# THU-DA-6D-Pose-Group/GDR-Net

Hardware: AMD Instinct MI355X
Metric: RoI crops/sec (fwd+bwd) at 256×256 bs=64 (higher is better)
Workload: dtype bf16; 1 GPU; LM-13 a6_cPnP_lm13 graph: ResNet-34 + RotWithRegionHead + ConvPnPNet, 256x256 RoIs, bs=64/GPU, train step: fwd + 8 losses + bwd + fused Ranger optimizer step (all inside the timed region); global_batch=64, parallelism=dp1

## Files before the change

### gdr-net_amd/cabi.py

```python
import ctypes as C
import os

_HERE = os.path.dirname(os.path.abspath(__file__))
LIB_PATH = os.environ.get("GDRN_HIP_LIB") or os.path.join(_HERE, "lib", "libgdrn_hip.so")
LIB_PATH_F16 = os.environ.get("GDRN_HIP_LIB_F16") or os.path.join(_HERE, "lib", "libgdrn_hip_f16.so")

F32, BF16, F16 = 0, 1, 2
PREZEROED = 0x100
ACC_ROWS = 0x200
P = C.c_void_p
I = C.c_int
LL = C.c_longlong
F = C.c_float
D = C.c_double


class GdrnHipError(RuntimeError):
    pass


class ConvParams(C.Structure):
    _fields_ = [
        ("x", P), ("w", P), ("y", P), ("bias", P), ("addend", P), ("stats", P),
        ("bnb_x", P), ("bnb_mask", P), ("bnb_mean", P), ("bnb_invstd", P), ("bnb_scale", P), ("bnb_shift", P), ("bnb_rows", P),
# ... 128 lines not shown
    "gdrn_stem_conv_pool": [P, P, P, P, P, I, I, P],
    "gdrn_head_conv_tail_fwd": [P, I, P, I, P, P, P, P, I, P, I, I, I, I, I, P],
    "gdrn_head_conv_tail_loss_rows": [I, I],
    "gdrn_head_out_dgrad_rows": [I, I],
    "gdrn_head_out_dgrad": [P, I, P, I, P, I, P, P, P, P, P, I, P, I, I, I, P],
    "gdrn_head_conv_tail_loss_fwd": [P, I, P, I, P, P, P, P, I, P, I, P, P, P, P, P, I, I, I, I, P],
    "gdrn_stem_wgrad_parts": [I],
    "gdrn_stem_wgrad": [P, P, P, P, P, P, I, P, P, I, P],
    "gdrn_linear_splitk": [P, P, P, P, I, I, I, I, I, I, I, P, I, P],
    "gdrn_conv_tile": [C.POINTER(ConvParams), C.POINTER(I), C.POINTER(I)],
    "gdrn_conv_stats_rows": [C.POINTER(ConvParams)],
    "gdrn_pack_wfrag": [P, P, I, I, I, P],
    "gdrn_pack_wfrag32": [P, P, I, I, I, P],
    "gdrn_conv3x3_wfrag": [C.POINTER(ConvParams)],
    "gdrn_conv3x3_halo": [C.POINTER(ConvParams), P],
    "gdrn_conv3x3_tile": [C.POINTER(ConvParams), C.POINTER(I), C.POINTER(I), C.POINTER(I)],
    "gdrn_conv3x3_stats_rows": [C.POINTER(ConvParams)],
    "gdrn_conv3x3_halo_waves": [C.POINTER(ConvParams)],
    "gdrn_conv_wgrad": [C.POINTER(WgradParams), P],
    "gdrn_conv3x3_wgrad": [C.POINTER(WgradParams), P],
    "gdrn_conv3x3_wgrad_ok": [C.POINTER(WgradParams)],
    "gdrn_conv3x3_wgrad_splits": [C.POINTER(WgradParams)],
    "gdrn_conv3x3_wgrad_multi": [P, P, I, I, P],
    "gdrn_conv3x3_wgrad_multi_lds": [P, P, I, I, I, P],
    "gdrn_wgrad_reduce_multi": [P, P, I, I, P],
    "gdrn_pack4": [P, P, I, I, I, I, I, I, I, LL, LL, LL, LL, I, I, P],
    "gdrn_unpack4": [P, P, I, I, I, I, I, I, I, LL, LL, LL, LL, I, P],
    "gdrn_pack_stem_w": [P, P, I, P],
    "gdrn_unpack_stem_w": [P, P, P],
    "gdrn_pack_image": [P, P, I, I, I, I, I, I, P],
    "gdrn_cast_from_f32": [P, P, LL, I, P],
    "gdrn_cast_to_f32": [P, P, LL, I, P],
    "gdrn_nhwc_to_nchw_f32": [P, I, I, I, P, I, I, I, P],
    "gdrn_bn_finalize": [P, I, I, D, P, P, P, P, P, F, F, P, P, P, P, P, P],
    "gdrn_bn_eval_params": [P, P, P, P, F, I, P, P, P],
    "gdrn_bn_apply": [P, P, P, P, P, LL, I, I, I, P],
    "gdrn_bn_bwd_reduce_rows": [LL, I, I],
    "gdrn_bn_bwd_reduce": [P, P, P, P, P, P, P, LL, I, P, I, P],
    "gdrn_bn_bwd_coef": [P, I, I, LL, P, P, P, P, P, P, P, P, P],
    "gdrn_bn_bwd_apply": [P, P, P, P, P, P, P, P, LL, I, P, P, I, P],
    "gdrn_bn_relu_maxpool_fwd": [P, P, P, P, P, I, I, I, I, I, P],
    "gdrn_maxpool_bwd_rows": [I, I, I, I, I],
    "gdrn_maxpool_bwd": [P, P, P, P, P, P, I, I, I, I, P, P, P, I, P],
    "gdrn_upsample2x_fwd": [P, P, I, I, I, I, I, P],
    "gdrn_upsample2x_bwd": [P, P, I, I, I, I, I, P],
    "gdrn_conv3x3s2_ok": [C.POINTER(S2Params)],
    "gdrn_conv3x3s2_stats_rows": [C.POINTER(S2Params)],
    "gdrn_conv3x3s2": [C.POINTER(S2Params), P],
    "gdrn_conv3x3s2_dgrad_ok": [C.POINTER(S2dParams)],
    "gdrn_conv3x3s2_dgrad_rows": [C.POINTER(S2dParams)],
    "gdrn_conv3x3s2_dgrad": [C.POINTER(S2dParams), P],
    "gdrn_block64_eval_ok": [I, I, I, I],
    "gdrn_block64_eval": [P, P, P, P, P, P, I, I, I, I, P],
    "gdrn_bn_relu_upsample2x_fwd": [P, P, P, P, I, I, I, I, I, P],
    "gdrn_upsample2x_bwd_bnsums": [P, P, P, P, P, P, P, I, I, I, I, P, I, P],
    "gdrn_gn_relu_fwd": [P, P, P, P, P, I, I, I, I, F, I, P],
    "gdrn_gn_relu_bwd": [P, P, P, P, P, P, P, P, I, I, I, I, I, P],
    "gdrn_leaky_bwd": [P, P, P, LL, I, P],
    "gdrn_bias_grad": [P, I, I, I, P, I, P],
    "gdrn_head_tail_fwd": [P, I, P, P, P, I, I, I, I, I, P],
    "gdrn_head_tail_loss_fwd": [P, I, P, P, P, I, P, P, P, P, P, I, I, I, I, P],
    "gdrn_map_loss_fwd": [P, I, P, P, P, P, I, I, I, P, P],
    "gdrn_map_loss_finalize": [P, I, I, P, P],
    "gdrn_head_tail_loss_rows": [I, I, I, I, I],
    "gdrn_map_loss_finalize_rows": [P, I, I, I, P, P],
    "gdrn_loss_finalize": [P, I, I, I, P, P, P, P, P],
    "gdrn_linear_splits": [I, I],
    "gdrn_head_tail_bwd": [P, I, P, P, I, P, P, P, P, P, P, P, P, I, I, I, I, I, P],
    "gdrn_pose_loss": [C.POINTER(PoseParams), P],
    "gdrn_combine3": [P, P, P, I, P],
    "gdrn_ranger_step": [P, P, P, P, P, I, I, I, F, F, F, F, F, F, I, I, F, P],
    "gdrn_pack_chunk": [],
    "gdrn_zero_chunk": [],
    "gdrn_zero_multi": [P, P, I, I, P],
    "gdrn_nonfinite_flag": [P, LL, P, P],
    "gdrn_pack_multi": [P, P, I, I, I, P],
    "gdrn_pack_transpose_blocks": [P],
    "gdrn_unpack_multi": [P, P, I, I, P],
    "gdrn_ranger_multi": [P, P, I, I, F, F, F, F, F, I, I, F, F, P],
    "gdrn_ranger_multi_dyn": [P, P, I, I, F, F, F, F, I, I, F, F, P, P],
    "gdrn_loss_scale_update": [P, I, P],
    "gdrn_unscale_or_zero": [P, LL, F, P, P],
    "gdrn_scaled_loss_weights": [P, P, I, P, P, P],
    "gdrn_roi_affine": [P, I, I, I, P, P, P, P, P],
    "gdrn_roi_crop_inputs": [P, P, I, I, I, C.POINTER(D), C.POINTER(D), P, P, P],
    "gdrn_roi_targets": [P, P, I, I, P, I, P, P, P, P, P, P, P],
    "gdrn_pose_metrics_workspace_bytes": [I, I],
    "gdrn_pose_errors": [P, P, P, P, P, P, P, I, P, P, I, P, P, P, I, I, P, P, P],
    "gdrn_pose_recall_accumulate": [P, P, P, I, P, I, P, P, P, P, P, P],
    "gdrn_pnp_workspace_bytes": [I, I, I],
    "gdrn_pnp_ransac": [P, P, P, P, P, I, I, D, I, C.c_ulonglong, I, P, P, P, P, P, P, P, P],
    "gdrn_pnp_refine": [P, P, P, P, P, I, I, I, P, P, P, P, P, P],
    "gdrn_pnp_ransac_f64": [P, P, P, P, P, I, I, D, I, C.c_ulonglong, I, P, P, P, P, P, P, P, P],
    "gdrn_pnp_refine_f64": [P, P, P, P, P, I, I, I, P, P, P, P, P, P],
    "gdrn_render_depth": [P, P, P, P, P, P, I, I, P, P, P, P, P, I, I, I, D, D, P, P],
    "gdrn_xyz_from_depth": [P, P, P, P, I, I, I, P, P, P, P, P],
    "gdrn_vsd_workspace_bytes": [I, I, I, I],
    "gdrn_vsd": [P, P, P, P, P, I, P, P, I, I, I, D, P, I, I, I, P, P, P, P],
    "gdrn_mssd_mspd_workspace_bytes": [I, I, I],
    "gdrn_mssd_mspd": [P, P, P, P, P, P, P, I, P, P, I, P, P, P, I, I, P, P, P],
    "gdrn_bop_recall_accumulate": [P, I, P, P, P, I, P, I, D, P, P, P, P, P, P, P, P],
    "gdrn_ad_errors_workspace_bytes": [I, I],
    "gdrn_ad_errors": [P, P, P, P, P, P, I, P, P, I, I, P, P, P],
    "gdrn_sym_errors_workspace_bytes": [I, I, I],
    "gdrn_sym_errors": [P, P, P, P, P, P, P, I, P, P, I, P, P, P, I, I, P, P, P],
    "gdrn_score_recall_accumulate": [P, P, P, P, I, P, P, I, P, P, P],
    "gdrn_aug_mask_cuts": [P, C.POINTER(AugTask), I, P, P],
    "gdrn_aug_frames": [P, C.POINTER(AugTask), I, P, LL, P, P],
    "gdrn_rle_decode": [P, C.POINTER(RleTask), I, P, LL, P, LL, P, P, P],
    "gdrn_rle_count": [P, C.POINTER(RleTask), I, P, LL, P, P, P],
    "gdrn_rle_positions": [P, C.POINTER(RleTask), I, P, LL, P, P, LL, P],
    "gdrn_rle_string": [P, C.POINTER(RleTask), I, P, P, LL, P, P, LL, P, P],
    "gdrn_model_prep_workspace_bytes": [I, I, I],
    "gdrn_model_bounds": [P, P, P, I, I, P, P],
    "gdrn_model_fps": [P, P, P, I, I, I, P, P, P, P],
    "gdrn_model_diameter": [P, P, P, I, I, P, P],
    "gdrn_scene_gt_canvas": [P, I, I, I, I, I, P, P, P, P],
    "gdrn_scene_gt_compose": [P, P, P, P, P, I, I, I, I, P, P],
    "gdrn_scene_gt_visibility": [P, P, P, P, I, P, I, I, I, D, I, P, P, P, P, P, P, P, P, P],
    "gdrn_render_visibility": [P, P, P, P, P, P, I, I, P, P, P, P, P, I, I, I, D, D, P, P],
    "gdrn_shade_frames": [P, P, P, P, P, P, P, P, P, I, P, P, P, P, P, P, P, P, P, I, I, I, I, P, P, P, P, P, P, P, P, P],
    "gdrn_shade_frames_tex": [P, P, P, P, P, P, P, P, P, P, P, P, P, I, I, P, P, P, P, P, P, P, P, P, I, I, I, I, P, P, I, I, P, P, P, P, P, P, P],
}

_SIGS["gdrn_half_format"] = []
_RET_LL = ("gdrn_workspace_bytes", "gdrn_pose_metrics_workspace_bytes", "gdrn_pnp_workspace_bytes", "gdrn_vsd_workspace_bytes",
           "gdrn_mssd_mspd_workspace_bytes", "gdrn_model_prep_workspace_bytes", "gdrn_ad_errors_workspace_bytes",
           "gdrn_sym_errors_workspace_bytes")
EXPORTS = tuple(_SIGS.keys())
_libs = {}


def lib_path(dtype=BF16):
    return LIB_PATH_F16 if dtype == F16 else LIB_PATH


def load(dtype=BF16):
    kind = F16 if dtype == F16 else BF16
    if kind in _libs:
        return _libs[kind]
    import torch

    path = lib_path(kind)
    if not os.path.exists(path):
        raise GdrnHipError(
            f"{path} not found: build it with `python -c 'import __graft_entry__ as g; g.build()'` "
            "(hipcc --offload-arch=gfx950).  There is no CPU fallback for the product path."
        )
    lib = C.CDLL(path)
    for name, args in _SIGS.items():
        fn = getattr(lib, name)
        fn.argtypes = args
        fn.restype = LL if name in _RET_LL else I
    if lib.gdrn_half_format() != kind:
        raise GdrnHipError(f"{path} computes 16-bit dtype code {lib.gdrn_half_format()}, expected {kind}")
    _libs[kind] = lib
    return lib


def check(status, what=""):
    if status != 0:
        names = {-1: "invalid argument", -2: "unsupported shape", -3: "launch failure"}
        detail = ""
        if status == -3:
            for lib in _libs.values():
                buf = C.create_string_buffer(64)
                code = lib.gdrn_last_hip_error(buf, 64)
                if code:
                    detail = f" (HIP error {code}: {buf.value.decode(errors='replace')})"
                    break
        raise GdrnHipError(f"libgdrn_hip: {what} failed: {names.get(status, status)}{detail}")


def ptr(t):
    return None if t is None else t.data_ptr()
```

### gdr-net_amd/csrc/conv3x3_halo.hip

```cpp
#include <hip/amd_detail/amd_hip_unsafe_atomics.h>

#include <algorithm>
#include <cstdlib>
#include <mutex>

#include "common.h"
#include "halo_xf.h"
#include "../../include/gdrn_hip.h"

namespace {

constexpr int ROWB = 128;

__device__ __forceinline__ f32x4_t mma_f32(uint4 a, uint4 b, f32x4_t c, int ks_) {
    const unsigned av = ks_ == 0 ? a.x : (ks_ == 1 ? a.y : (ks_ == 2 ? a.z : a.w));
    const unsigned bv = ks_ == 0 ? b.x : (ks_ == 1 ? b.y : (ks_ == 2 ? b.z : b.w));
    return __builtin_amdgcn_mfma_f32_16x16x4f32(__uint_as_float(av), __uint_as_float(bv), c, 0, 0, 0);
}

template <typename T>
__global__ __launch_bounds__(256) void pack_wfrag_kernel(const T* __restrict__ src, T* __restrict__ dst, int rows, int Cin) {
    constexpr int EPS = ROWB / (int)sizeof(T);
    constexpr int GE = 16 / (int)sizeof(T);
    const int kch = Cin / EPS;
    const long long total = (long long)rows * 9 * Cin / GE;
    for (long long i = (long long)blockIdx.x * blockDim.x + threadIdx.x; i < total; i += (long long)gridDim.x * blockDim.x) {
        const int lane = (int)(i & 63);
        long long r = i >> 6;
        const int ks = (int)(r & 1); r >>= 1;
        const int kc = (int)(r % kch); r /= kch;
        const int tap = (int)(r % 9);
        const int cb = (int)(r / 9);
        const int FNp = (rows <= 64 || sizeof(T) == 4) ? 1 : 2, rr = lane & 15;
        const int co = (cb / FNp) * 16 * FNp + (rr >> 2) * (4 * FNp) + (cb % FNp) * 4 + (rr & 3), g = lane >> 4;
        const size_t so = ((size_t)(co * 9 + tap) * Cin + (size_t)kc * EPS) + (size_t)(ks * 4 + g) * GE;
        *reinterpret_cast<uint4*>(dst + i * GE) = *reinterpret_cast<const uint4*>(src + so);
    }
}

#ifdef HALO_DBG
__device__ unsigned long long* g_halo_dbg;
__device__ __forceinline__ unsigned long long halo_clock() {
    unsigned long long t;
    asm volatile("s_memtime %0\n\ts_waitcnt lgkmcnt(0)" : "=s"(t)::"memory");
    return t;
}
struct HaloDbg {
    unsigned long long t[6] = {0, 0, 0, 0, 0, 0};
    int slot, lane;
    __device__ ~HaloDbg() {
        t[4] = halo_clock();
        asm volatile("s_waitcnt vmcnt(0)" ::: "memory");
        t[5] = halo_clock();
        if (lane == 0 && g_halo_dbg)
            for (int i = 0; i < 6; ++i) g_halo_dbg[(size_t)slot * 8 + i] = t[i];
    }
};
extern "C" int gdrn_halo_set_dbg(unsigned long long* buf) { return hipMemcpyToSymbol(HIP_SYMBOL(g_halo_dbg), &buf, sizeof(buf)) == hipSuccess ? 0 : -3; }
#define HALO_STAMP(i_) hdbg_.t[i_] = halo_clock();
#else
#define HALO_STAMP(i_)
#endif

template <typename T, int TH, int TW, int BN, int XF, int KS = 1>
__global__ __launch_bounds__(256 * KS, KS == 2 ? 1 : ((BN == 64 && TW == 16 && sizeof(T) == 2) ? 3 : 2)) void conv3x3_halo_kernel(const gdrn_conv_params p) {
    static_assert(KS == 1 || (KS == 2 && sizeof(T) == 2 && BN == 128), "the 8-wave form: 16-bit, 128-channel tile");
    constexpr int EPS = ROWB / (int)sizeof(T);
    constexpr int BM = TH * TW;
    constexpr int PW = TW + 2, PH = TH + 2, PPIX = PH * PW;
    constexpr int HB = half_bytes(PPIX);
    constexpr int PBYTES = 2 * HB;
    constexpr int PSEG = PPIX * 8;
    constexpr int PSLICE = XF ? ((PSEG + 8) / 9 + 7) / 8 * 8 : (PSEG + 8) / 9;
    static_assert(PSLICE <= 256, "one patch segment per thread per stage");
    static_assert(XF == 0 || sizeof(T) == 2, "operand transforms are bf16 only");
    constexpr int FM = BM / 16;
    constexpr int FN = BN / 64;
    constexpr int WQ = FN * 2 / KS;
    constexpr int NSL = KS == 2 ? 5 : 9;
    extern __shared__ __attribute__((aligned(16))) unsigned char smem[];

    const int lane = threadIdx.x & 63;
    const int grp = KS == 2 ? __builtin_amdgcn_readfirstlane((int)threadIdx.x >> 8) : 0;
    const int tid = threadIdx.x & 255, wave = tid >> 6;
    const int g = lane >> 4, r16 = lane & 15;
#ifdef HALO_DBG
    HaloDbg hdbg_;
    hdbg_.slot = (int)blockIdx.x * 4 + wave;
    hdbg_.lane = lane;
#endif
    HALO_STAMP(0)
    __builtin_amdgcn_s_setprio(2);

    const int NTn = (p.Cout + BN - 1) / BN;
    int bid = blockIdx.x;
    {
        const int nwg = gridDim.x, q = nwg >> 3, r = nwg & 7, xcd = bid & 7, j = bid >> 3;
        bid = (xcd < r ? xcd * (q + 1) : r * (q + 1) + (xcd - r) * q) + j;
    }
    const int nt = bid % NTn;
    const int mt = bid / NTn;
    int t = mt;
    const int tiles_x = p.Wo / TW, tiles_y = p.Ho / TH;
    const int tx = t % tiles_x; t /= tiles_x;
    const int ty = t % tiles_y;
    const int n = t / tiles_y;
    const int co0 = nt * BN;
    const int y0 = ty * TH, x0 = tx * TW;

    const int kch = p.Cin / EPS;
    const char* xg = reinterpret_cast<const char*>(p.x);
    const int cb0 = (co0 + wave * (BN / 4)) / 16;
    const char* wl = reinterpret_cast<const char*>(p.w) + (size_t)lane * 16 + (size_t)(grp << 10);

    auto wptr = [&](int kc, int tap, int a, int ks) -> const uint4* {
        return reinterpret_cast<const uint4*>(wl + ((size_t)((((cb0 + a) * 9 + tap) * kch + kc) * 2 + ks) << 10));
    };
    uint4 wq0[WQ], wq1[WQ], wq2[WQ];

#define LOADW(dst, kc_, tap_)                                                   \
    {                                                                           \
        _Pragma("unroll") for (int a_ = 0; a_ < FN; ++a_) {                     \
            if constexpr (KS == 1) {                                            \
                dst[a_ * 2 + 0] = *wptr(kc_, tap_, a_, 0);                      \
                dst[a_ * 2 + 1] = *wptr(kc_, tap_, a_, 1);                      \
            } else dst[a_] = *wptr(kc_, tap_, a_, 0);                           \
        }                                                                       \
    }
    LOADW(wq0, 0, 0) LOADW(wq1, 0, 1) LOADW(wq2, 0, 2)

    unsigned poff[NSL];
    int pdst[NSL];
    unsigned pokm = 0, pinm = 0, ppm = 0;
#pragma unroll
    for (int sj = 0; sj < NSL; ++sj) {
        const int st = KS == 2 ? 2 * sj + grp : sj;
        const int id = st * PSLICE + tid;
        const int pp = id >> 3, sg = id & 7;
        const int py = pp / PW, px = pp - py * PW;
        const int iy = y0 + py - 1, ix = x0 + px - 1;
        const bool inpatch = tid < PSLICE && id < PSEG && st < 9;
        const bool ok = inpatch && iy >= 0 && iy < p.Hi && ix >= 0 && ix < p.Wi;
        const int iyc = min(max(iy, 0), p.Hi - 1), ixc = min(max(ix, 0), p.Wi - 1);
        poff[sj] = (unsigned)((n * p.Hi + iyc) * p.Wi + ixc) * (unsigned)p.x_cs * (unsigned)sizeof(T) + sg * 16;
        pdst[sj] = inpatch ? (pp * HALF_PITCH + (sg & 1) * HB + (sg >> 1) * 16) : -1;
        pokm |= ok ? (1u << sj) : 0u;
        if constexpr (XF != 0) {
            pinm |= (inpatch && py >= 1 && py <= TH && px >= 1 && px <= TW) ? (1u << sj) : 0u;
            ppm |= inpatch ? (1u << sj) : 0u;
        }
    }
    constexpr int PDSTEP = (PSLICE / 8) * HALF_PITCH;
    const int pdst0 = (tid >> 3) * HALF_PITCH + (tid & 1) * HB + ((tid & 7) >> 1) * 16 + grp * PDSTEP;
#define OWN(st_) (KS == 1 || (((st_) & 1) == grp))
#define SJ(st_) (KS == 1 ? (st_) : ((st_) >> 1))
    const float* xtab = nullptr;
    const char* xg2 = nullptr;
    char* xo = nullptr;
    float xlo = 0.f;
    if constexpr (XF != 0) {
        float* tabw = reinterpret_cast<float*>(smem + (kch == 1 ? 1 : 2) * PBYTES);
        for (int c = (int)threadIdx.x; c < p.Cin; c += 256 * KS) {
            tabw[c] = p.xf_a ? p.xf_a[c] : 1.f;
            tabw[p.Cin + c] = p.xf_c[c];
            if constexpr (XF >= 2) tabw[2 * p.Cin + c] = p.xf_b ? p.xf_b[c] : 1.f;
            if constexpr (XF == 2) tabw[3 * p.Cin + c] = p.xf_c2 ? p.xf_c2[c] : 0.f;
            if constexpr (XF == 4) { tabw[3 * p.Cin + c] = p.xf_msc[c]; tabw[4 * p.Cin + c] = p.xf_msh[c]; }
        }
        xtab = tabw + (tid & 7) * 8;
        xg2 = reinterpret_cast<const char*>(p.xf_x2);
        xo = (nt == 0) ? reinterpret_cast<char*>(p.xf_out) : nullptr;
        xlo = p.xf_relu ? 0.f : -__builtin_inff();
    }

    int lbase;
    if constexpr (TW == 16) lbase = r16 * HALF_PITCH + (g & 1) * HB + (g >> 1) * 16;
    else lbase = ((r16 >> 3) * PW + (r16 & 7)) * HALF_PITCH + (g & 1) * HB + (g >> 1) * 16;
    lbase += grp * 32;
    constexpr int FROW = (TW == 16) ? PW * HALF_PITCH : 2 * PW * HALF_PITCH;

    f32x4_t acc[FN][FM];
#pragma unroll
    for (int a = 0; a < FN; ++a)
#pragma unroll
        for (int b = 0; b < FM; ++b) acc[a][b] = f32x4_t{0.f, 0.f, 0.f, 0.f};
    f32x4_t part[sizeof(T) == 4 ? FN : 1][sizeof(T) == 4 ? FM : 1];

    uint4 rp0 = make_uint4(0, 0, 0, 0), rp1 = rp0, rp2 = rp0;
    uint4 rq0 = rp0, rq1 = rp0, rq2 = rp0;
#define RP(i_) (((i_) % 3) == 0 ? rp0 : (((i_) % 3) == 1 ? rp1 : rp2))
#define RQ(i_) (((i_) % 3) == 0 ? rq0 : (((i_) % 3) == 1 ? rq1 : rq2))

#define LOADP(dst, dst2, kc_, st_)                                              \
    if (OWN(st_)) {                                                             \
        const uint4 v_ = *reinterpret_cast<const uint4*>(xg + (poff[SJ(st_)] + (unsigned)((kc_) * ROWB))); \
        if constexpr (XF == 0) dst = ((pokm >> SJ(st_)) & 1u) ? v_ : make_uint4(0, 0, 0, 0);          \
        else dst = v_;                                                          \
        if constexpr (XF >= 2) dst2 = *reinterpret_cast<const uint4*>(xg2 + (poff[SJ(st_)] + (unsigned)((kc_) * ROWB))); \
    }
#define WRITEP(src, src2, pb_, st_, kc_)                                        \
    if (OWN(st_)) {                                                             \
        if constexpr (XF == 0) {                                                \
            if (pdst[SJ(st_)] >= 0) *reinterpret_cast<uint4*>(smem + (pb_) * PBYTES + pdst[SJ(st_)]) = src; \
        } else {                                                                \
            if ((ppm >> SJ(st_)) & 1u) {                                        \
                uint4 t_ = xf_apply<XF>(src, src2, xtab + (kc_) * EPS, p.Cin, xlo); \
                t_ = ((pokm >> SJ(st_)) & 1u) ? t_ : make_uint4(0, 0, 0, 0);   \
                *reinterpret_cast<uint4*>(smem + (pb_) * PBYTES + pdst0 + SJ(st_) * (PDSTEP * KS)) = t_; \
                if (xo != nullptr && ((pinm >> SJ(st_)) & 1u))                  \
                    *reinterpret_cast<uint4*>(xo + (poff[SJ(st_)] + (unsigned)((kc_) * ROWB))) = t_; \
            }                                                                   \
        }                                                                       \
    }

    {
        uint4 q0, q1, q2, q3, q4, q5, q6, q7, q8;
        uint4 u0 = rp0, u1 = rp0, u2 = rp0, u3 = rp0, u4 = rp0, u5 = rp0, u6 = rp0, u7 = rp0, u8 = rp0;
        LOADP(q0, u0, 0, 0) LOADP(q1, u1, 0, 1) LOADP(q2, u2, 0, 2) LOADP(q3, u3, 0, 3) LOADP(q4, u4, 0, 4)
        LOADP(q5, u5, 0, 5) LOADP(q6, u6, 0, 6) LOADP(q7, u7, 0, 7) LOADP(q8, u8, 0, 8)
        if constexpr (XF != 0) __syncthreads();
        WRITEP(q0, u0, 0, 0, 0) WRITEP(q1, u1, 0, 1, 0) WRITEP(q2, u2, 0, 2, 0) WRITEP(q3, u3, 0, 3, 0) WRITEP(q4, u4, 0, 4, 0)
        WRITEP(q5, u5, 0, 5, 0) WRITEP(q6, u6, 0, 6, 0) WRITEP(q7, u7, 0, 7, 0) WRITEP(q8, u8, 0, 8, 0)
    }
    HALO_STAMP(1)
    __syncthreads();
    HALO_STAMP(2)

    uint4 fbA[FM], fbB[FM];
#define RD(dst_, TAP_, KS_)                                                                                     \
    {                                                                                                           \
        constexpr int tsh_ = ((TAP_) / 3) * PW * HALF_PITCH + ((TAP_) % 3) * HALF_PITCH;                        \
        _Pragma("unroll") for (int b_ = 0; b_ < FM; ++b_)                                                       \
            dst_[b_] = *reinterpret_cast<const uint4*>(pcur + (b_ * FROW + tsh_ + (KS_) * 32));                 \
    }
#define MM(WQ_, KS_, src_)                                                                                      \
    {                                                                                                           \
        if constexpr (sizeof(T) == 4) {                                                                         \
            _Pragma("unroll") for (int k4_ = 0; k4_ < 4; ++k4_)                                                 \
                _Pragma("unroll") for (int a_ = 0; a_ < FN; ++a_)                                               \
                    _Pragma("unroll") for (int b_ = 0; b_ < FM; ++b_)                                           \
                        part[a_][b_] = mma_f32(WQ_[a_ * 2 + (KS_)], src_[b_], part[a_][b_], k4_);               \
        } else {                                                                                                \
            _Pragma("unroll") for (int a_ = 0; a_ < FN; ++a_)                                                   \
                _Pragma("unroll") for (int b_ = 0; b_ < FM; ++b_)                                               \
                    acc[a_][b_] = mma_step<T>(WQ_[a_ * (2 / KS) + (KS_)], src_[b_], acc[a_][b_]);               \
        }                                                                                                       \
    }
#define STEP(WQ_, TAP_)                                                                                         \
    {                                                                                                           \
        if (more_p) {                                                                                           \
            if constexpr ((TAP_) >= 2) WRITEP(RP((TAP_) + 1), RQ((TAP_) + 1), pb ^ 1, (TAP_) - 2, kc + 1)       \
            if constexpr ((TAP_) == 0) { LOADP(rp0, rq0, kc + 1, 0) LOADP(rp1, rq1, kc + 1, 1) }                \
            else if constexpr ((TAP_) <= 7) LOADP(RP((TAP_) + 1), RQ((TAP_) + 1), kc + 1, (TAP_) + 1)           \
        }                                                                                                       \
        if constexpr (KS == 2) {         \
            if constexpr ((TAP_) < 8) {                                                                         \
                if constexpr ((TAP_) & 1) RD(fbA, (TAP_) + 1, 0) else RD(fbB, (TAP_) + 1, 0)                    \
            }                                                                                                   \
            if constexpr ((TAP_) & 1) MM(WQ_, 0, fbB) else MM(WQ_, 0, fbA)                                      \
        } else {                                                                                                \
        RD(fbB, TAP_, 1)                                                                                        \
        if constexpr (sizeof(T) == 4) {                                                                         \
            _Pragma("unroll") for (int a_ = 0; a_ < FN; ++a_)                                                   \
                _Pragma("unroll") for (int b_ = 0; b_ < FM; ++b_) part[a_][b_] = f32x4_t{0.f, 0.f, 0.f, 0.f};   \
        }                                                                                                       \
        MM(WQ_, 0, fbA)                                                                                         \
        \
        if constexpr ((TAP_) < 8) RD(fbA, (TAP_) + 1, 0)                                                        \
        \
        MM(WQ_, 1, fbB)                                                                                         \
        if constexpr (sizeof(T) == 4) {                                                                         \
            _Pragma("unroll") for (int a_ = 0; a_ < FN; ++a_)                                                   \
                _Pragma("unroll") for (int b_ = 0; b_ < FM; ++b_) acc[a_][b_] += part[a_][b_];                  \
        }                                                                                                       \
        }                                                                                                       \
        {                                                                                                       \
            constexpr int nt_ = ((TAP_) + 3) % 9;                                                               \
            const int nk_ = kc + (((TAP_) + 3) >= 9 ? 1 : 0);                                                   \
            if (nk_ < kch) LOADW(WQ_, nk_, nt_)                                                                 \
        }                                                                                                       \
    }

    for (int kc = 0; kc < kch; ++kc) {
        const int pb = kc & 1;
        const bool more_p = kc + 1 < kch;
        const unsigned char* pcur = smem + pb * PBYTES + lbase;
        RD(fbA, 0, 0)
        STEP(wq0, 0) STEP(wq1, 1) STEP(wq2, 2)
        STEP(wq0, 3) STEP(wq1, 4) STEP(wq2, 5)
        STEP(wq0, 6) STEP(wq1, 7) STEP(wq2, 8)
        if (more_p) { WRITEP(rp1, rq1, pb ^ 1, 7, kc + 1) WRITEP(rp2, rq2, pb ^ 1, 8, kc + 1) }
        __syncthreads();
    }
    HALO_STAMP(3)
#undef LOADW
#undef LOADP
#undef WRITEP
#undef RD
#undef MM
#undef STEP
#undef RP
#undef RQ
#undef OWN
#undef SJ

    if constexpr (KS == 2) {
        float4* ex = reinterpret_cast<float4*>(smem) + wave * (FN * FM * 64) + lane;
        if (grp == 1) {
#pragma unroll
            for (int a = 0; a < FN; ++a)
#pragma unroll
                for (int b = 0; b < FM; ++b) ex[(a * FM + b) * 64] = make_float4(acc[a][b][0], acc[a][b][1], acc[a][b][2], acc[a][b][3]);
        }
        __syncthreads();
        if (grp == 1) return;
#pragma unroll
        for (int a = 0; a < FN; ++a)
#pragma unroll
            for (int b = 0; b < FM; ++b) {
                const float4 o = ex[(a * FM + b) * 64];
                acc[a][b][0] += o.x; acc[a][b][1] += o.y; acc[a][b][2] += o.z; acc[a][b][3] += o.w;
            }
    }

    if constexpr (sizeof(T) == 2) {
        if (p.act <= 1 && !p.out_f32 && (p.Cout % BN) == 0) {
            const int cl = co0 + wave * (BN / 4) + g * (4 * FN);
            auto ld_ch = [&](const char* base, unsigned elem_off, uint2 (&dst)[FN]) {
                if constexpr (FN == 2) {
                    const uint4 q = *reinterpret_cast<const uint4*>(base + elem_off * 2u);
                    dst[0] = make_uint2(q.x, q.y);
                    dst[1] = make_uint2(q.z, q.w);
                } else {
#pragma unroll
                    for (int a = 0; a < FN; ++a) dst[a] = *reinterpret_cast<const uint2*>(base + (elem_off + (unsigned)(a * 4)) * 2u);
                }
            };
            auto st_ch = [&](char* base, unsigned elem_off, const uint2 (&src)[FN]) {
                if constexpr (FN == 2) {
                    *reinterpret_cast<uint4*>(base + elem_off * 2u) = make_uint4(src[0].x, src[0].y, src[1].x, src[1].y);
                } else {
#pragma unroll
                    for (int a = 0; a < FN; ++a) *reinterpret_cast<uint2*>(base + (elem_off + (unsigned)(a * 4)) * 2u) = src[a];
                }
            };
            if (p.stats != nullptr) {
                float* srow = p.stats + (size_t)mt * 2 * p.Cout + cl;
#pragma unroll
                for (int a = 0; a < FN; ++a) {
                    float s1[4], s2[4];
#pragma unroll
                    for (int j = 0; j < 4; ++j) {
                        float u = 0.f, q = 0.f;
#pragma unroll
                        for (int b = 0; b < FM; ++b) { const float v = acc[a][b][j]; u += v; q += v * v; }
                        s1[j] = row16_sum(u);
                        s2[j] = row16_sum(q);
                    }
                    if (r16 == 0) {
                        *reinterpret_cast<float4*>(srow + a * 4) = make_float4(s1[0], s1[1], s1[2], s1[3]);
                        *reinterpret_cast<float4*>(srow + p.Cout + a * 4) = make_float4(s2[0], s2[1], s2[2], s2[3]);
                    }
                }
            }
            const int prow0 = (n * p.Ho + y0 + (TW == 16 ? 0 : (r16 >> 3))) * p.Wo + x0 + (TW == 16 ? r16 : (r16 & 7));
            const int pstep = (TW == 16 ? 1 : 2) * p.Wo;
            char* yb = reinterpret_cast<char*>(p.y);
            const char* ab = reinterpret_cast<const char*>(p.addend);
            if (p.bnb_x != nullptr) {
                const char* xb = reinterpret_cast<const char*>(p.bnb_x);
                const char* mb = reinterpret_cast<const char*>(p.bnb_mask);
                const bool affine = mb == nullptr && p.bnb_scale != nullptr;
                float kmu[FN][4], kis[FN][4], ksc[FN][4], ksh[FN][4], t1[FN][4], t2[FN][4];
#pragma unroll
                for (int a = 0; a < FN; ++a) {
                    const float4 mu = *reinterpret_cast<const float4*>(p.bnb_mean + cl + a * 4);
                    const float4 is = *reinterpret_cast<const float4*>(p.bnb_invstd + cl + a * 4);
                    kmu[a][0] = mu.x; kmu[a][1] = mu.y; kmu[a][2] = mu.z; kmu[a][3] = mu.w;
                    kis[a][0] = is.x; kis[a][1] = is.y; kis[a][2] = is.z; kis[a][3] = is.w;
                    float4 sc = make_float4(0.f, 0.f, 0.f, 0.f), sh = make_float4(1.f, 1.f, 1.f, 1.f);
                    if (affine) {
                        sc = *reinterpret_cast<const float4*>(p.bnb_scale + cl + a * 4);
                        sh = *reinterpret_cast<const float4*>(p.bnb_shift + cl + a * 4);
                    }
                    ksc[a][0] = sc.x; ksc[a][1] = sc.y; ksc[a][2] = sc.z; ksc[a][3] = sc.w;
                    ksh[a][0] = sh.x; ksh[a][1] = sh.y; ksh[a][2] = sh.z; ksh[a][3] = sh.w;
#pragma unroll
                    for (int j = 0; j < 4; ++j) { t1[a][j] = 0.f; t2[a][j] = 0.f; }
                }
                constexpr int HB_ = FM / 2;
#pragma unroll
                for (int h = 0; h < 2; ++h) {
                    uint2 xq[HB_][FN], av[HB_][FN], mq[HB_][FN];
#pragma unroll
                    for (int bb = 0; bb < HB_; ++bb) {
                        const unsigned pr = (unsigned)(prow0 + (h * HB_ + bb) * pstep);
                        ld_ch(xb, pr * (unsigned)p.bnb_cs + (unsigned)cl, xq[bb]);
#pragma unroll
                        for (int a = 0; a < FN; ++a) {
                            av[bb][a] = make_uint2(0u, 0u);
                            mq[bb][a] = make_uint2(GDRN_H16_ONE2, GDRN_H16_ONE2);
                        }
                    }
                    if (ab != nullptr) {
#pragma unroll
                        for (int bb = 0; bb < HB_; ++bb) {
                            const unsigned pr = (unsigned)(prow0 + (h * HB_ + bb) * pstep);
                            ld_ch(ab, pr * (unsigned)p.add_cs + (unsigned)cl, av[bb]);
                        }
                    }
                    if (mb != nullptr) {
#pragma unroll
                        for (int bb = 0; bb < HB_; ++bb) {
                            const unsigned pr = (unsigned)(prow0 + (h * HB_ + bb) * pstep);
                            ld_ch(mb, pr * (unsigned)p.bnb_cs + (unsigned)cl, mq[bb]);
                        }
                    }
#pragma unroll
                    for (int bb = 0; bb < HB_; ++bb) {
                        const int b = h * HB_ + bb;
                        const unsigned pr = (unsigned)(prow0 + b * pstep);
                        uint2 ov[FN];
#pragma unroll
                        for (int a = 0; a < FN; ++a) {
                            const uint2 xw = xq[bb][a], aw = av[bb][a], mw = mq[bb][a];
                            const float xv[4] = {h16lo(xw.x), h16hi(xw.x),
                                                 h16lo(xw.y), h16hi(xw.y)};
                            const float mv[4] = {h16lo(mw.x), h16hi(mw.x),
                                                 h16lo(mw.y), h16hi(mw.y)};
                            const float ad[4] = {h16lo(aw.x), h16hi(aw.x),
                                                 h16lo(aw.y), h16hi(aw.y)};
                            float v[4];
#pragma unroll
                            for (int j = 0; j < 4; ++j) {
                                const bool keep = (mv[j] > 0.f) && (xv[j] * ksc[a][j] + ksh[a][j] > 0.f);
                                const float gv = keep ? acc[a][b][j] + ad[j] : 0.f;
                                v[j] = gv;
                                t1[a][j] += gv;
                                t2[a][j] += gv * (xv[j] - kmu[a][j]) * kis[a][j];
                            }
                            ov[a] = make_uint2(pack_bf2(v[0], v[1]), pack_bf2(v[2], v[3]));
                        }
                        st_ch(yb, pr * (unsigned)p.y_cs + (unsigned)cl, ov);
                    }
                }
                float* srow = p.bnb_rows + (size_t)mt * 2 * p.Cout + cl;
#pragma unroll
                for (int a = 0; a < FN; ++a) {
                    float u1[4], u2[4];
#pragma unroll
                    for (int j = 0; j < 4; ++j) { u1[j] = row16_sum(t1[a][j]); u2[j] = row16_sum(t2[a][j]); }
                    if (r16 == 0) {
                        *reinterpret_cast<float4*>(srow + a * 4) = make_float4(u1[0], u1[1], u1[2], u1[3]);
                        *reinterpret_cast<float4*>(srow + p.Cout + a * 4) = make_float4(u2[0], u2[1], u2[2], u2[3]);
                    }
                }
                return;
            }
            float bq[FN][4];
#pragma unroll
            for (int a = 0; a < FN; ++a) {
                float4 bv = make_float4(0.f, 0.f, 0.f, 0.f);
                if (p.bias != nullptr) bv = *reinterpret_cast<const float4*>(p.bias + cl + a * 4);
                bq[a][0] = bv.x; bq[a][1] = bv.y; bq[a][2] = bv.z; bq[a][3] = bv.w;
            }
            const bool relu = p.act == 1;
            if (ab != nullptr) {
                uint2 avq[FM][FN];
#pragma unroll
                for (int b = 0; b < FM; ++b) {
                    const unsigned pr = (unsigned)(prow0 + b * pstep);
                    ld_ch(ab, pr * (unsigned)p.add_cs + (unsigned)cl, avq[b]);
                }
#pragma unroll
                for (int b = 0; b < FM; ++b) {
                    const unsigned pr = (unsigned)(prow0 + b * pstep);
                    uint2 ov[FN];
#pragma unroll
                    for (int a = 0; a < FN; ++a) {
                        const uint2 av_ = avq[b][a];
                        float v0 = acc[a][b][0] + bq[a][0] + h16lo(av_.x), v1 = acc[a][b][1] + bq[a][1] + h16hi(av_.x);
                        float v2 = acc[a][b][2] + bq[a][2] + h16lo(av_.y), v3 = acc[a][b][3] + bq[a][3] + h16hi(av_.y);
                        if (relu) { v0 = fmaxf(v0, 0.f); v1 = fmaxf(v1, 0.f); v2 = fmaxf(v2, 0.f); v3 = fmaxf(v3, 0.f); }
                        ov[a] = make_uint2(pack_bf2(v0, v1), pack_bf2(v2, v3));
                    }
                    st_ch(yb, pr * (unsigned)p.y_cs + (unsigned)cl, ov);
                }
            } else {
#pragma unroll
                for (int b = 0; b < FM; ++b) {
                    const unsigned pr = (unsigned)(prow0 + b * pstep);
                    uint2 ov[FN];
#pragma unroll
                    for (int a = 0; a < FN; ++a) {
                        float v0 = acc[a][b][0] + bq[a][0], v1 = acc[a][b][1] + bq[a][1], v2 = acc[a][b][2] + bq[a][2], v3 = acc[a][b][3] + bq[a][3];
                        if (relu) { v0 = fmaxf(v0, 0.f); v1 = fmaxf(v1, 0.f); v2 = fmaxf(v2, 0.f); v3 = fmaxf(v3, 0.f); }
                        ov[a] = make_uint2(pack_bf2(v0, v1), pack_bf2(v2, v3));
                    }
                    st_ch(yb, pr * (unsigned)p.y_cs + (unsigned)cl, ov);
                }
            }
            return;
        }
    }
    if (p.stats != nullptr) {
#pragma unroll
        for (int a = 0; a < FN; ++a) {
#pragma unroll
            for (int j = 0; j < 4; ++j) {
                float s1 = 0.f, s2 = 0.f;
#pragma unroll
                for (int b = 0; b < FM; ++b) { const float v = acc[a][b][j]; s1 += v; s2 += v * v; }
#pragma unroll
                for (int o = 8; o > 0; o >>= 1) { s1 += __shfl_xor(s1, o, 64); s2 += __shfl_xor(s2, o, 64); }
                const int c = co0 + wave * (BN / 4) + g * (4 * FN) + a * 4 + j;
                if (r16 == 0 && c < p.Cout) {
                    p.stats[((size_t)mt * 2 + 0) * p.Cout + c] = s1;
                    p.stats[((size_t)mt * 2 + 1) * p.Cout + c] = s2;
                }
            }
        }
    }

#pragma unroll
    for (int b = 0; b < FM; ++b) {
        const int m = b * 16 + r16;
        const size_t orow = (size_t)(n * p.Ho + y0 + m / TW) * p.Wo + x0 + (m % TW);
#pragma unroll
        for (int a = 0; a < FN; ++a) {
            const int c0 = co0 + wave * (BN / 4) + g * (4 * FN) + a * 4;
            if (c0 >= p.Cout) continue;
            float v[4];
#pragma unroll
            for (int j = 0; j < 4; ++j) v[j] = acc[a][b][j];
            const bool full = (c0 + 3 < p.Cout);
            if (p.bias != nullptr) {
#pragma unroll
                for (int j = 0; j < 4; ++j) if (c0 + j < p.Cout) v[j] += p.bias[c0 + j];
            }
            if (p.addend != nullptr) {
                const T* ap = reinterpret_cast<const T*>(p.addend) + orow * p.add_cs + c0;
#pragma unroll
                for (int j = 0; j < 4; ++j) if (c0 + j < p.Cout) v[j] += ld1<T>(ap + j);
            }
            if (p.act == 1) {
#pragma unroll
                for (int j = 0; j < 4; ++j) v[j] = fmaxf(v[j], 0.f);
            } else if (p.act == 2) {
#pragma unroll
                for (int j = 0; j < 4; ++j) v[j] = v[j] > 0.f ? v[j] : 0.1f * v[j];
            }
            if (p.out_f32 || sizeof(T) == 4) {
                float* yp = reinterpret_cast<float*>(p.y) + orow * p.y_cs + c0;
                if (full) *reinterpret_cast<float4*>(yp) = make_float4(v[0], v[1], v[2], v[3]);
                else
#pragma unroll
                    for (int j = 0; j < 4; ++j) if (c0 + j < p.Cout) yp[j] = v[j];
            } else {
                bf16_t* yp = reinterpret_cast<bf16_t*>(p.y) + orow * p.y_cs + c0;
                if (full) *reinterpret_cast<uint2*>(yp) = make_uint2(pack_bf2(v[0], v[1]), pack_bf2(v[2], v[3]));
                else
#pragma unroll
                    for (int j = 0; j < 4; ++j) if (c0 + j < p.Cout) yp[j] = f2bf(v[j]);
            }
        }
    }
}

constexpr int XF_MAX_CIN = 512;

template <typename T, int TH, int TW, int BN, int XF, int KS = 1>
int launch(const gdrn_conv_params& p, int N, hipStream_t st) {
    constexpr size_t smem = 2 * 2 * (size_t)half_bytes((TH + 2) * (TW + 2));
    constexpr size_t xbytes = KS == 2 ? (size_t)4 * (BN / 64) * (TH * TW / 16) * 64 * 16 : 0;
    constexpr size_t smem_max = std::max(smem + xf_nk(XF) * XF_MAX_CIN * sizeof(float), xbytes);
    static std::once_flag attr_once;
    static bool attr_ok = false;
    std::call_once(attr_once, [] {
        attr_ok = hipFuncSetAttribute(reinterpret_cast<const void*>(&conv3x3_halo_kernel<T, TH, TW, BN, XF, KS>),
                                      hipFuncAttributeMaxDynamicSharedMemorySize, (int)smem_max) == hipSuccess;
    });
    if (!attr_ok) return GDRN_ERR_LAUNCH;
    const int grid = N * (p.Ho / TH) * (p.Wo / TW) * cdiv(p.Cout, BN);
    const size_t smem_used = std::max(((p.Cin * (int)sizeof(T) == ROWB) ? smem / 2 : smem) + (size_t)xf_nk(XF) * p.Cin * sizeof(float), xbytes);
    GDRN_LAUNCH((conv3x3_halo_kernel<T, TH, TW, BN, XF, KS>), dim3(grid), dim3(256 * KS), smem_used, st, p);
    GDRN_CHECK_LAUNCH();
    return GDRN_OK;
}

__host__ inline bool halo_split(const gdrn_conv_params& p, int th, int tw, int bn, int N) {
    if (bn != 128 || p.dtype != GDRN_DT_H16 || p.halo_waves == 4) return false;
    if (p.halo_waves == 8) return true;
    return (long long)N * (p.Ho / th) * (p.Wo / tw) * cdiv(p.Cout, bn) <= 256;
}

template <int XF>
int launch_tile(const gdrn_conv_params& p, int tw, int bn, int N, hipStream_t st) {
    if (halo_split(p, 8, tw, bn, N)) return tw == 16 ? launch<bf16_t, 8, 16, 128, XF, 2>(p, N, st) : launch<bf16_t, 8, 8, 128, XF, 2>(p, N, st);
    if (tw == 16) return bn == 64 ? launch<bf16_t, 8, 16, 64, XF>(p, N, st) : launch<bf16_t, 8, 16, 128, XF>(p, N, st);
    return bn == 64 ? launch<bf16_t, 8, 8, 64, XF>(p, N, st) : launch<bf16_t, 8, 8, 128, XF>(p, N, st);
}

int launch_tile_f32(const gdrn_conv_params& p, int tw, int N, hipStream_t st) {
    return tw == 8 ? launch<float, 8, 8, 64, 0>(p, N, st) : GDRN_ERR_SHAPE;
}

}

int gdrn_v3_config(const gdrn_conv_params* p);
int gdrn_v3_preferred(const gdrn_conv_params* p);
int gdrn_v3_tile(const gdrn_conv_params* p, int* th, int* tw, int* bn);
int gdrn_v3_launch(const gdrn_conv_params* p, void* stream);

extern "C" int gdrn_conv3x3_wfrag(const gdrn_conv_params* p) {
    if (!p) return GDRN_ERR_ARG;
    if (p->w_frag < 0 || p->w_frag > 2) return GDRN_ERR_ARG;
    if (p->w_frag == 2 && gdrn_v3_config(p) > 0) return 2;
    if (p->w_frag == 0 && gdrn_v3_preferred(p)) return 2;
    gdrn_conv_params q = *p;
    q.w_frag = 0;
    int th, tw, bn;
    gdrn_conv3x3_tile(&q, &th, &tw, &bn);
    return th > 0 ? 1 : 0;
}

extern "C" int gdrn_conv3x3_tile(const gdrn_conv_params* p, int* th, int* tw, int* bn) {
    if (!p || !th || !tw || !bn) return GDRN_ERR_ARG;
    *th = *tw = *bn = 0;
    if (p->w_frag == 2) { gdrn_v3_tile(p, th, tw, bn); return GDRN_OK; }
    if (p->mode != 0 || p->KH != 3 || p->KW != 3 || p->stride != 1 || p->pad != 1 || p->Hi != p->Ho || p->Wi != p->Wo) return GDRN_OK;
    if ((p->Ho % 8) || (p->Wo % 8)) return GDRN_OK;
    if (p->dtype != GDRN_DT_H16 && p->dtype != GDRN_DT_F32) return GDRN_OK;
    *th = 8;
    *tw = (p->Wo % 16 == 0 && p->dtype != GDRN_DT_F32) ? 16 : 8;
    *bn = (p->Cout <= 64 || p->dtype == GDRN_DT_F32) ? 64 : 128;
    return GDRN_OK;
}

extern "C" int gdrn_conv3x3_halo_waves(const gdrn_conv_params* p) {
    if (!p || p->w_frag == 2) return 0;
    int th, tw, bn;
    if (gdrn_conv3x3_tile(p, &th, &tw, &bn) != GDRN_OK || th == 0) return 0;
    return halo_split(*p, th, tw, bn, p->M / (p->Ho * p->Wo)) ? 8 : 4;
}

extern "C" int gdrn_conv3x3_stats_rows(const gdrn_conv_params* p) {
    int th, tw, bn;
    if (gdrn_conv3x3_tile(p, &th, &tw, &bn) != GDRN_OK || th == 0) return GDRN_ERR_SHAPE;
    const int hw = p->Ho * p->Wo;
    return (p->M / hw) * (p->Ho / th) * (p->Wo / tw);
}

extern "C" int gdrn_pack_wfrag(const void* src, void* dst, int rows, int Cin, int dtype, void* stream) {
    if (!src || !dst || rows <= 0 || (rows % 16) || Cin <= 0) return GDRN_ERR_ARG;
    const int esz = dtype == GDRN_DT_H16 ? 2 : 4;
    if ((Cin * esz) % ROWB) return GDRN_ERR_SHAPE;
    const long long n = (long long)rows * 9 * Cin * esz / 16;
    const int grid = (int)std::min<long long>((n + 255) / 256, 4096);
    hipStream_t st = reinterpret_cast<hipStream_t>(stream);
    if (dtype == GDRN_DT_F32) GDRN_LAUNCH(pack_wfrag_kernel<float>, dim3(grid), dim3(256), 0, st, (const float*)src, (float*)dst, rows, Cin);
    else if (dtype == GDRN_DT_H16) GDRN_LAUNCH(pack_wfrag_kernel<bf16_t>, dim3(grid), dim3(256), 0, st, (const bf16_t*)src, (bf16_t*)dst, rows, Cin);
    else return GDRN_ERR_ARG;
    GDRN_CHECK_LAUNCH();
    return GDRN_OK;
}

extern "C" int gdrn_conv3x3_halo(const gdrn_conv_params* pp, void* stream) {
    if (!pp || !pp->x || !pp->w || !pp->y) return GDRN_ERR_ARG;
    const gdrn_conv_params& p = *pp;
    if (p.dtype != GDRN_DT_F32 && p.dtype != GDRN_DT_H16) return GDRN_ERR_ARG;
    if (p.w_frag == 2) return gdrn_v3_launch(pp, stream);
    const int esz = p.dtype == GDRN_DT_H16 ? 2 : 4;
    int th, tw, bn;
    gdrn_conv3x3_tile(pp, &th, &tw, &bn);
    if (th == 0) return GDRN_ERR_SHAPE;
    if (p.Cin <= 0 || (p.Cin * esz) % ROWB != 0 || (p.x_cs * esz) % 16 != 0 || p.Cout <= 0 || (p.y_cs & 3)) return GDRN_ERR_SHAPE;
    if (bn == 128 && ((p.y_cs & 7) || (p.addend && (p.add_cs & 7)) || (p.bnb_x && (p.bnb_cs & 7)))) return GDRN_ERR_SHAPE;
    const int hw = p.Ho * p.Wo;
    if (p.M <= 0 || p.M % hw != 0) return GDRN_ERR_SHAPE;
    if (p.w_rows < cdiv(p.Cout, bn) * bn) return GDRN_ERR_SHAPE;
    if (p.addend && (p.add_cs & 3)) return GDRN_ERR_SHAPE;
    if (p.w_frag < 0 || p.w_frag > 2) return GDRN_ERR_ARG;
    if (p.halo_waves != 0 && p.halo_waves != 4 && p.halo_waves != 8) return GDRN_ERR_ARG;
    if (p.bnb_x) {
        if (!p.bnb_mean || !p.bnb_invstd || !p.bnb_rows || (p.bnb_scale != nullptr) != (p.bnb_shift != nullptr)) return GDRN_ERR_ARG;
        if (p.bias || p.act || p.out_f32 || (p.Cout % bn) || (p.bnb_cs & 3) || p.bnb_cs < p.Cout) return GDRN_ERR_SHAPE;
        if ((unsigned long long)p.M * (unsigned long long)p.bnb_cs * 4ull >= (1ull << 32)) return GDRN_ERR_SHAPE;
    }
    if ((unsigned long long)p.M * (unsigned long long)std::max(p.y_cs, p.add_cs) * 4ull >= (1ull << 32)) return GDRN_ERR_SHAPE;
    if ((unsigned long long)p.M * (unsigned long long)p.x_cs * (unsigned long long)esz >= (1ull << 32)) return GDRN_ERR_SHAPE;
    if (p.dtype == GDRN_DT_F32 && (p.xf_mode || p.bnb_x)) return GDRN_ERR_ARG;
    if (p.xf_mode) {
        if (p.xf_mode < 0 || p.xf_mode > 4 || !p.xf_c || p.Cin > XF_MAX_CIN || (p.Cin & 7)) return GDRN_ERR_ARG;
        if (p.xf_mode >= 2 && !p.xf_x2) return GDRN_ERR_ARG;
        if (p.xf_mode == 4 && (!p.xf_msc || !p.xf_msh)) return GDRN_ERR_ARG;
        if (p.xf_mode != 2 && p.xf_c2) return GDRN_ERR_ARG;
    }
    const int N = p.M / hw;
    hipStream_t st = reinterpret_cast<hipStream_t>(stream);
    if (p.dtype == GDRN_DT_F32) return launch_tile_f32(p, tw, N, st);
    switch (p.xf_mode) {
        case 0: return launch_tile<0>(p, tw, bn, N, st);
        case 1: return launch_tile<1>(p, tw, bn, N, st);
        case 2: return launch_tile<2>(p, tw, bn, N, st);
        case 3: return launch_tile<3>(p, tw, bn, N, st);
        default: return launch_tile<4>(p, tw, bn, N, st);
    }
}
```

Baseline: 9422 RoI/s.

## Add low-register 64-channel halo conv3x3 kernel variant for Cin=64 layers

Adds a specialised 3x3 halo convolution path for 8x16-pixel, 64-output-channel bf16 tiles whose input has exactly 64 channels. The new kernel is launched with 4 blocks per CU instead of 3. Its inner loop streams half-fragment LDS reads in a ping-pong pattern interleaved with MFMAs under sched barriers, and it defers some weight and patch loads so fewer registers are live at once. This targets occupancy and latency hiding in the ResNet-34 stem-stage convolutions. It is on by default, can be switched off with an env var, and risks register spills or worse instruction scheduling.

```diff
diff --git a/gdr-net_amd/cabi.py b/gdr-net_amd/cabi.py
--- a/gdr-net_amd/cabi.py
+++ b/gdr-net_amd/cabi.py
@@ -304,6 +304,12 @@
         fn = getattr(lib, name)
         fn.argtypes = args
         fn.restype = LL if name in _RET_LL else I
+    v = os.environ.get("GDRN_HALO64_LOWREG")
+    if v is not None:
+        if v not in ("0", "1"):
+            raise ValueError("GDRN_HALO64_LOWREG must be 0 or 1, not %r" % v)
+        if hasattr(lib, "gdrn_conv3x3_halo64_lowreg"):
+            lib.gdrn_conv3x3_halo64_lowreg(int(v))
     if lib.gdrn_half_format() != kind:
         raise GdrnHipError(f"{path} computes 16-bit dtype code {lib.gdrn_half_format()}, expected {kind}")
     _libs[kind] = lib
diff --git a/gdr-net_amd/csrc/conv3x3_halo.hip b/gdr-net_amd/csrc/conv3x3_halo.hip
--- a/gdr-net_amd/csrc/conv3x3_halo.hip
+++ b/gdr-net_amd/csrc/conv3x3_halo.hip
@@ -1,6 +1,7 @@
 #include <hip/amd_detail/amd_hip_unsafe_atomics.h>
 
 #include <algorithm>
+#include <atomic>
 #include <cstdlib>
 #include <mutex>
 
@@ -62,9 +63,10 @@
 #define HALO_STAMP(i_)
 #endif
 
-template <typename T, int TH, int TW, int BN, int XF, int KS = 1>
-__global__ __launch_bounds__(256 * KS, KS == 2 ? 1 : ((BN == 64 && TW == 16 && sizeof(T) == 2) ? 3 : 2)) void conv3x3_halo_kernel(const gdrn_conv_params p) {
+template <typename T, int TH, int TW, int BN, int XF, int KS, int LR>
+__device__ __forceinline__ void conv3x3_halo_body(const gdrn_conv_params& p) {
     static_assert(KS == 1 || (KS == 2 && sizeof(T) == 2 && BN == 128), "the 8-wave form: 16-bit, 128-channel tile");
+    static_assert(LR == 0 || (KS == 1 && sizeof(T) == 2 && BN == 64 && TH == 8 && TW == 16), "the low-register form: 16-bit, 8x16 pixels x 64 channels");
     constexpr int EPS = ROWB / (int)sizeof(T);
     constexpr int BM = TH * TW;
     constexpr int PW = TW + 2, PH = TH + 2, PPIX = PH * PW;
@@ -108,7 +110,7 @@
     const int co0 = nt * BN;
     const int y0 = ty * TH, x0 = tx * TW;
 
-    const int kch = p.Cin / EPS;
+    const int kch = LR ? 1 : p.Cin / EPS;
     const char* xg = reinterpret_cast<const char*>(p.x);
     const int cb0 = (co0 + wave * (BN / 4)) / 16;
     const char* wl = reinterpret_cast<const char*>(p.w) + (size_t)lane * 16 + (size_t)(grp << 10);
@@ -127,7 +129,9 @@
             } else dst[a_] = *wptr(kc_, tap_, a_, 0);                           \
         }                                                                       \
     }
-    LOADW(wq0, 0, 0) LOADW(wq1, 0, 1) LOADW(wq2, 0, 2)
+    constexpr bool WLATE = LR && XF >= 2;
+    LOADW(wq0, 0, 0)
+    if constexpr (!WLATE) { LOADW(wq1, 0, 1) LOADW(wq2, 0, 2) }
 
     unsigned poff[NSL];
     int pdst[NSL];
@@ -149,6 +153,11 @@
             pinm |= (inpatch && py >= 1 && py <= TH && px >= 1 && px <= TW) ? (1u << sj) : 0u;
             ppm |= inpatch ? (1u << sj) : 0u;
         }
+    }
+    if constexpr (LR) {
+#pragma unroll
+        for (int sj = 0; sj < NSL; ++sj) asm volatile("" : "+v"(poff[sj]));
+        asm volatile("" : "+v"(pokm), "+v"(pinm), "+v"(ppm));
     }
     constexpr int PDSTEP = (PSLICE / 8) * HALF_PITCH;
     const int pdst0 = (tid >> 3) * HALF_PITCH + (tid & 1) * HB + ((tid & 7) >> 1) * 16 + grp * PDSTEP;
@@ -210,6 +219,8 @@
                 if (xo != nullptr && ((pinm >> SJ(st_)) & 1u))                  \
                     *reinterpret_cast<uint4*>(xo + (poff[SJ(st_)] + (unsigned)((kc_) * ROWB))) = t_; \
             }                                                                   \
+             \
+            if constexpr (LR) asm volatile("" ::: "memory");                    \
         }                                                                       \
     }
 
@@ -217,10 +228,18 @@
         uint4 q0, q1, q2, q3, q4, q5, q6, q7, q8;
         uint4 u0 = rp0, u1 = rp0, u2 = rp0, u3 = rp0, u4 = rp0, u5 = rp0, u6 = rp0, u7 = rp0, u8 = rp0;
         LOADP(q0, u0, 0, 0) LOADP(q1, u1, 0, 1) LOADP(q2, u2, 0, 2) LOADP(q3, u3, 0, 3) LOADP(q4, u4, 0, 4)
-        LOADP(q5, u5, 0, 5) LOADP(q6, u6, 0, 6) LOADP(q7, u7, 0, 7) LOADP(q8, u8, 0, 8)
+        LOADP(q5, u5, 0, 5) LOADP(q6, u6, 0, 6)
+        constexpr int PLATE = !WLATE ? 0 : (XF == 2 ? 2 : 1);
+        if constexpr (PLATE < 2) LOADP(q7, u7, 0, 7)
+        if constexpr (PLATE < 1) LOADP(q8, u8, 0, 8)
         if constexpr (XF != 0) __syncthreads();
-        WRITEP(q0, u0, 0, 0, 0) WRITEP(q1, u1, 0, 1, 0) WRITEP(q2, u2, 0, 2, 0) WRITEP(q3, u3, 0, 3, 0) WRITEP(q4, u4, 0, 4, 0)
+        WRITEP(q0, u0, 0, 0, 0)
+        if constexpr (PLATE == 2) LOADP(q7, u7, 0, 7)
+        if constexpr (PLATE == 1) LOADP(q8, u8, 0, 8)
+        WRITEP(q1, u1, 0, 1, 0)
+        if constexpr (PLATE == 2) LOADP(q8, u8, 0, 8) WRITEP(q2, u2, 0, 2, 0) WRITEP(q3, u3, 0, 3, 0) WRITEP(q4, u4, 0, 4, 0)
         WRITEP(q5, u5, 0, 5, 0) WRITEP(q6, u6, 0, 6, 0) WRITEP(q7, u7, 0, 7, 0) WRITEP(q8, u8, 0, 8, 0)
+        if constexpr (WLATE) { LOADW(wq1, 0, 1) LOADW(wq2, 0, 2) }
     }
     HALO_STAMP(1)
     __syncthreads();
@@ -281,6 +300,41 @@
         }                                                                                                       \
     }
 
+    if constexpr (LR) {
+        constexpr int FH = FM / 2;
+        const unsigned char* pcur = smem + lbase;
+        uint4 fa[FH], fb[FH];
+#define RDH(dst_, TAP_, KS_, H_)                                                                                \
+    {                                                                                                           \
+        constexpr int tsh_ = ((TAP_) / 3) * PW * HALF_PITCH + ((TAP_) % 3) * HALF_PITCH;                        \
+        _Pragma("unroll") for (int b_ = 0; b_ < FH; ++b_)                                                       \
+            dst_[b_] = *reinterpret_cast<const uint4*>(pcur + (((H_) * FH + b_) * FROW + tsh_ + (KS_) * 32));   \
+        __builtin_amdgcn_sched_barrier(0);                                                                      \
+    }
+#define MMH(WQ_, KS_, src_, H_)                                                                                 \
+    {                                                                                                           \
+        _Pragma("unroll") for (int b_ = 0; b_ < FH; ++b_)                                                       \
+            acc[0][(H_) * FH + b_] = mma_step<T>(WQ_[KS_], src_[b_], acc[0][(H_) * FH + b_]);                   \
+        __builtin_amdgcn_sched_barrier(0);                                                                      \
+    }
+#define STEPL(WQ_, TAP_)                                                                                        \
+    {                                                                                                           \
+        RDH(fb, TAP_, 0, 1) MMH(WQ_, 0, fa, 0)                                                                  \
+        RDH(fa, TAP_, 1, 0) MMH(WQ_, 0, fb, 1)                                                                  \
+        RDH(fb, TAP_, 1, 1) MMH(WQ_, 1, fa, 0)                                                                  \
+        if constexpr ((TAP_) < 8) RDH(fa, (TAP_) + 1, 0, 0)                                                     \
+        MMH(WQ_, 1, fb, 1)                                                                                      \
+        if constexpr ((TAP_) + 3 < 9) { LOADW(WQ_, 0, (TAP_) + 3) __builtin_amdgcn_sched_barrier(0); }          \
+    }
+        __builtin_amdgcn_sched_barrier(0);
+        RDH(fa, 0, 0, 0)
+        STEPL(wq0, 0) STEPL(wq1, 1) STEPL(wq2, 2)
+        STEPL(wq0, 3) STEPL(wq1, 4) STEPL(wq2, 5)
+        STEPL(wq0, 6) STEPL(wq1, 7) STEPL(wq2, 8)
+#undef RDH
+#undef MMH
+#undef STEPL
+    } else
     for (int kc = 0; kc < kch; ++kc) {
         const int pb = kc & 1;
         const bool more_p = kc + 1 < kch;
@@ -567,23 +621,40 @@
     }
 }
 
+template <typename T, int TH, int TW, int BN, int XF, int KS = 1>
+__global__ __launch_bounds__(256 * KS, KS == 2 ? 1 : ((BN == 64 && TW == 16 && sizeof(T) == 2) ? 3 : 2)) void conv3x3_halo_kernel(const gdrn_conv_params p) {
+    conv3x3_halo_body<T, TH, TW, BN, XF, KS, 0>(p);
+}
+
+template <typename T, int XF>
+__global__ __launch_bounds__(256, 4) void conv3x3_halo64_kernel(const gdrn_conv_params p) {
+    conv3x3_halo_body<T, 8, 16, 64, XF, 1, 1>(p);
+}
+
 constexpr int XF_MAX_CIN = 512;
 
-template <typename T, int TH, int TW, int BN, int XF, int KS = 1>
+template <typename T, int TH, int TW, int BN, int XF, int KS, int LR>
+constexpr auto halo_entry() -> void (*)(const gdrn_conv_params) {
+    if constexpr (LR) return &conv3x3_halo64_kernel<T, XF>;
+    else return &conv3x3_halo_kernel<T, TH, TW, BN, XF, KS>;
+}
+
+template <typename T, int TH, int TW, int BN, int XF, int KS = 1, int LR = 0>
 int launch(const gdrn_conv_params& p, int N, hipStream_t st) {
     constexpr size_t smem = 2 * 2 * (size_t)half_bytes((TH + 2) * (TW + 2));
     constexpr size_t xbytes = KS == 2 ? (size_t)4 * (BN / 64) * (TH * TW / 16) * 64 * 16 : 0;
     constexpr size_t smem_max = std::max(smem + xf_nk(XF) * XF_MAX_CIN * sizeof(float), xbytes);
     static std::once_flag attr_once;
     static bool attr_ok = false;
-    std::call_once(attr_once, [] {
-        attr_ok = hipFuncSetAttribute(reinterpret_cast<const void*>(&conv3x3_halo_kernel<T, TH, TW, BN, XF, KS>),
+    void (*const kern)(const gdrn_conv_params) = halo_entry<T, TH, TW, BN, XF, KS, LR>();
+    std::call_once(attr_once, [kern] {
+        attr_ok = hipFuncSetAttribute(reinterpret_cast<const void*>(kern),
                                       hipFuncAttributeMaxDynamicSharedMemorySize, (int)smem_max) == hipSuccess;
     });
     if (!attr_ok) return GDRN_ERR_LAUNCH;
     const int grid = N * (p.Ho / TH) * (p.Wo / TW) * cdiv(p.Cout, BN);
     const size_t smem_used = std::max(((p.Cin * (int)sizeof(T) == ROWB) ? smem / 2 : smem) + (size_t)xf_nk(XF) * p.Cin * sizeof(float), xbytes);
-    GDRN_LAUNCH((conv3x3_halo_kernel<T, TH, TW, BN, XF, KS>), dim3(grid), dim3(256 * KS), smem_used, st, p);
+    GDRN_LAUNCH(kern, dim3(grid), dim3(256 * KS), smem_used, st, p);
     GDRN_CHECK_LAUNCH();
     return GDRN_OK;
 }
@@ -594,9 +665,13 @@
     return (long long)N * (p.Ho / th) * (p.Wo / tw) * cdiv(p.Cout, bn) <= 256;
 }
 
+std::atomic<int> g_halo64_lowreg{1};
+inline bool halo64_lowreg() { return g_halo64_lowreg.load(std::memory_order_relaxed) != 0; }
+
 template <int XF>
 int launch_tile(const gdrn_conv_params& p, int tw, int bn, int N, hipStream_t st) {
     if (halo_split(p, 8, tw, bn, N)) return tw == 16 ? launch<bf16_t, 8, 16, 128, XF, 2>(p, N, st) : launch<bf16_t, 8, 8, 128, XF, 2>(p, N, st);
+    if (tw == 16 && bn == 64 && p.Cin * (int)sizeof(bf16_t) == ROWB && halo64_lowreg()) return launch<bf16_t, 8, 16, 64, XF, 1, 1>(p, N, st);
     if (tw == 16) return bn == 64 ? launch<bf16_t, 8, 16, 64, XF>(p, N, st) : launch<bf16_t, 8, 16, 128, XF>(p, N, st);
     return bn == 64 ? launch<bf16_t, 8, 8, 64, XF>(p, N, st) : launch<bf16_t, 8, 8, 128, XF>(p, N, st);
 }
@@ -642,6 +717,11 @@
     int th, tw, bn;
     if (gdrn_conv3x3_tile(p, &th, &tw, &bn) != GDRN_OK || th == 0) return 0;
     return halo_split(*p, th, tw, bn, p->M / (p->Ho * p->Wo)) ? 8 : 4;
+}
+
+extern "C" int gdrn_conv3x3_halo64_lowreg(int on) {
+    if (on >= 0) g_halo64_lowreg.store(on ? 1 : 0, std::memory_order_relaxed);
+    return halo64_lowreg() ? 1 : 0;
 }
 
 extern "C" int gdrn_conv3x3_stats_rows(const gdrn_conv_params* p) {
```

Measured after the change: 9458 RoI/s, median of 3. About the same (+0.4%).
